# learningmatter-mit/surface-sampling

Hardware: AMD Instinct MI355X
Metric: MC energy-evaluations/sec (SrTiO3(001) ~250-atom slabs, 3-model PaiNN ensemble E+F incl. neighbor list) (higher is better)
Workload: dtype f32 via fp16x2-split MFMA (3 products), fp32 accumulate; neighbor decisions f64; 1 GPU; SrTiO3(001) PaiNN x3, 256 batched independent chains per GPU (BASELINE configs[3]), 248-272 atoms/chain; chains_per_gpu=256, atoms_per_gpu=66503, edges_per_gpu=2747786, slots_per_gpu=2836316, models=3, streams_per_gpu=2, parallelism=one GPU, no collective

## Files before the change

surface-sampling_amd/csrc/painn_edge_mfma.hip:

```cpp
#include "vssr_internal.h"

#ifdef EDGE_PHASE_TIMING
__device__ unsigned long long g_edge_phase[16];
#define EPH_INIT unsigned long long eph_acc[8] = {0, 0, 0, 0, 0, 0, 0, 0}, eph_t = wall_clock64();
#define EPH(k) { __builtin_amdgcn_sched_barrier(0); const unsigned long long eph_n = wall_clock64(); eph_acc[k] += eph_n - eph_t; eph_t = eph_n; __builtin_amdgcn_sched_barrier(0); }
#define EPH_FLUSH(base) if ((threadIdx.x & 63) == 0) { for (int q_ = 0; q_ < 8; ++q_) atomicAdd(&g_edge_phase[(base) + q_], eph_acc[q_]); }
extern "C" int vssr_debug_edge_phases(unsigned long long *out, int reset) {
    if (hipMemcpyFromSymbol(out, HIP_SYMBOL(g_edge_phase), sizeof(unsigned long long) * 16) != hipSuccess) return -1;
    if (reset) { unsigned long long z[16] = {}; if (hipMemcpyToSymbol(HIP_SYMBOL(g_edge_phase), z, sizeof(z)) != hipSuccess) return -1; }
    return 0;
}
#else
#define EPH_INIT
#define EPH(k)
#define EPH_FLUSH(base)
#endif

#ifndef SUB16_WAVES
#define SUB16_WAVES 12
#endif

namespace vssr {

typedef float f32x4 __attribute__((ext_vector_type(4)));

typedef unsigned u32x4 __attribute__((ext_vector_type(4)));
typedef _Float16 f16x8 __attribute__((ext_vector_type(8)));

__device__ __forceinline__ void mfma_pre_fence(u32x4 &a, u32x4 &b) {
    asm volatile("; mfma_pre_fence" : "+v"(a), "+v"(b) : : "memory");
}
__device__ __forceinline__ void arrival_fence(u32x4 &a, u32x4 &b) {
    asm volatile("; arrival_fence" : "+v"(a), "+v"(b) : : "memory");
}
__device__ __forceinline__ void arrival_fence(u32x4 &a, u32x4 &b, u32x4 &c, u32x4 &d, float &g) {
    asm volatile("; arrival_fence" : "+v"(a), "+v"(b), "+v"(c), "+v"(d), "+v"(g) : : "memory");
}
__device__ __forceinline__ float take(float src) {
    float d;
    asm("v_mov_b32 %0, %1" : "=v"(d) : "v"(src));
    return d;
}
__device__ __forceinline__ unsigned take_u(unsigned src) {
    unsigned d;
    asm("v_mov_b32 %0, %1" : "=v"(d) : "v"(src));
    return d;
}
__device__ __forceinline__ void mfma_load_fence(int &index, float &a, float &b, float &c) {
    asm volatile("; mfma_load_fence" : "+v"(index), "+v"(a), "+v"(b), "+v"(c));
}
// ... 54 lines not shown
    const auto hi = __builtin_amdgcn_permlane16_swap(a[1], a[1], false, false);
    s0 = __uint_as_float(lo[0]); s1 = __uint_as_float(lo[1]); s2 = __uint_as_float(hi[0]); s3 = __uint_as_float(hi[1]);
}

void build_wd16(const float *Wd, const float *bd, unsigned *dst) {
    auto split2 = [](float x, unsigned (&p)[2]) {
        const _Float16 h = (_Float16)x;
        const _Float16 l = (_Float16)(x - (float)h);
        unsigned short hb, lb;
        memcpy(&hb, &h, 2);
        memcpy(&lb, &l, 2);
        p[0] = hb; p[1] = lb;
    };
    for (int row = 0; row < F3; ++row)
        for (int kq = 0; kq < 4; ++kq) {
            unsigned wh[5], wl[5], bp[2];
            for (int t = 0; t < 5; ++t) {
                unsigned p2[2];
                split2(Wd[(size_t)row * 20 + kq + 4 * t], p2);
                wh[t] = p2[0]; wl[t] = p2[1];
            }
            split2(bd[row], bp);
            const unsigned bias = kq == 1 ? bp[1] : kq == 3 ? 0u : bp[0];
            const unsigned a1[8] = {wh[0], wh[1], wh[2], wh[3], wh[4], bias, wl[0], wl[1]};
            const unsigned a2[8] = {wl[2], wl[3], wl[4], wh[4], wh[0], wh[1], wh[2], wh[3]};
            unsigned *o = dst + ((size_t)row * 4 + kq) * 8;
            for (int q = 0; q < 4; ++q) {
                o[q] = a1[2 * q] | (a1[2 * q + 1] << 16);
                o[4 + q] = a2[2 * q] | (a2[2 * q + 1] << 16);
            }
        }
}

#ifndef STAGE_BATCH
#define STAGE_BATCH 4
#endif

template <int N> struct FeatVec { typedef float type __attribute__((ext_vector_type(N))); };
struct FeatVec1 {
    float v;
    __device__ __forceinline__ float operator[](int) const { return v; }
};
template <> struct FeatVec<1> { typedef FeatVec1 type; };

template <int NF>
struct EdgeGeo {
    static_assert(NF == 4 || NF == 2 || NF == 1, "16-, 8- or 4-feature slices");
    static constexpr int FS = 4 * NF;
    static constexpr int NSLICE = F / FS;
    static constexpr int NSEC = 3;
    static constexpr int NT = NF == 4 ? 3 : NF == 2 ? 2 : 1;
    static constexpr int NSEG = 6;
    static constexpr int ROW = NSEG * FS + 4;
    static constexpr int ROWB = FS * 4 + 4;
    __host__ __device__ static constexpr int row_section(int T, int i) {
        return NF == 4 ? T : NF == 1 ? ((i & 3) < 3 ? (i & 3) : -1) : (2 * T + ((i & 3) >> 1) < 3 ? 2 * T + ((i & 3) >> 1) : -1);
    }
    __host__ __device__ static constexpr int row_feature(int i) { return NF == 4 ? i : NF == 1 ? (i >> 2) : 2 * (i >> 2) + (i & 1); }
};
template <int NF> __device__ __forceinline__ constexpr int sec_tile(int sec) { return NF == 4 ? sec : NF == 1 ? 0 : sec >> 1; }
template <int NF> __device__ __forceinline__ constexpr int sec_reg(int sec, int r) { return NF == 4 ? r : NF == 1 ? sec : 2 * (sec & 1) + r; }

template <int NF, bool SLDS>
size_t edge_fwd_lds_bytes_t(int max_atoms) {
    return sizeof(float) * ((size_t)max_atoms * (EdgeGeo<NF>::ROW + (SLDS ? EdgeGeo<NF>::FS : 0)) + 4);
}

typedef float f32x2v __attribute__((ext_vector_type(2)));
// ... 20 lines not shown
}
template <int NF>
__device__ __forceinline__ void quad_sum_n(float (&x)[NF]) {
#pragma unroll
    for (int r = 0; r < NF; ++r) x[r] = quad_sum(x[r]);
    if constexpr (NF == 4) asm volatile("" : "+v"(x[0]), "+v"(x[1]), "+v"(x[2]), "+v"(x[3]));
    else if constexpr (NF == 2) asm volatile("" : "+v"(x[0]), "+v"(x[1]));
    else asm volatile("" : "+v"(x[0]));
}
template <int NF>
__device__ __forceinline__ void store_feat(float *dst, const float (&v)[NF]) {
    if constexpr (NF == 4) *reinterpret_cast<float4 *>(dst) = make_float4(v[0], v[1], v[2], v[3]);
    else if constexpr (NF == 2) *reinterpret_cast<float2 *>(dst) = make_float2(v[0], v[1]);
    else *dst = v[0];
}

__device__ __forceinline__ float xrow_sum(float x) {
    const unsigned u = __float_as_uint(x);
    const auto r32 = __builtin_amdgcn_permlane32_swap(u, u, false, false);
    const float y = __uint_as_float(r32[0]) + __uint_as_float(r32[1]);
    const unsigned v = __float_as_uint(y);
    const auto r16 = __builtin_amdgcn_permlane16_swap(v, v, false, false);
    return __uint_as_float(r16[0]) + __uint_as_float(r16[1]);
}

template <int NW>
struct BundleWalk {
    const int4 *tab;
    int Nc, wave, st;
    int nj;
    int j, t, Lc, Ln;
    int4 cur, nxt, pend;
    bool pend_ok;

    __device__ __forceinline__ int bundle_of(int jj) const { return jj * NW + ((jj & 1) ? NW - 1 - wave : wave); }
    __device__ __forceinline__ int4 load(int jj, bool &ok) const {
        const int idx = 4 * bundle_of(jj) + st;
        ok = jj < nj && idx < Nc;
        return tab[max(min(idx, Nc - 1), 0)];
    }
    __device__ __forceinline__ static int4 select(const int4 &v, bool ok) { return ok ? v : make_int4(-1, 0, 0, 0); }
    __device__ __forceinline__ static int steps(const int4 &q) { return max(__builtin_amdgcn_readfirstlane(q.z) >> 2, 2); }
    __device__ __forceinline__ void init(const int4 *table, int n, int w, int stream) {
        tab = table; Nc = n; wave = w; st = stream;
#ifdef ABL_NO_TAIL
        const int NB0 = (n + 3) >> 2, NB = NB0 >= NW ? NB0 - NB0 % NW : NB0, full = NB / NW, rem = NB - full * NW;
#else
        const int NB = (n + 3) >> 2, full = NB / NW, rem = NB - full * NW;
#endif
        nj = full + ((((full & 1) ? NW - 1 - w : w) < rem) ? 1 : 0);
        j = 0; t = 0;
        bool ok0, ok1;
        const int4 r0 = load(0, ok0), r1 = load(1, ok1);
        pend = load(2, pend_ok);
        cur = select(r0, ok0); nxt = select(r1, ok1);
        Lc = steps(cur); Ln = steps(nxt);
    }
    __device__ __forceinline__ int quad_ahead(int ahead, bool &valid) const {
        const int tt = t + ahead;
        const bool in_cur = tt < Lc;
        const int4 &q = in_cur ? cur : nxt;
        const int ts = in_cur ? tt : tt - Lc;
        valid = 4 * ts < q.z;
        return q.y + 4 * ts;
    }
    __device__ __forceinline__ void advance() {
        ++j;
        cur = nxt; nxt = select(pend, pend_ok);
        pend = load(j + 2, pend_ok);
        t = 0; Lc = Ln; Ln = steps(nxt);
    }
};

__device__ __forceinline__ int chain_of_workgroup(const GraphView &G, const int *__restrict__ list, int n_list, int per_chain, int &t) {
    const int wg = blockIdx.x, xcd = wg & 7, rest = wg >> 3;
    t = rest % per_chain;
    const int k = (rest / per_chain) * 8 + xcd;
    if (k >= n_list) return -1;
    const int b = list ? list[k] : k;
    return G.act.chain(b) ? b : -1;
}

template <bool ALIASED> struct EdgeOut { typedef float *__restrict__ ptr; };
template <> struct EdgeOut<true> { typedef float *ptr; };

template <int NF, bool SLDS, int WAVES, bool SUB = false>
__global__ void __launch_bounds__(64 * WAVES) __attribute__((amdgpu_waves_per_eu((SUB && NF == 4) ? WAVES / 4 : 4, (SUB && NF == 4) ? WAVES / 4 : 4)))
k_edge_fwd_mfma(int N, int l, const ModelW *__restrict__ MW, GraphView G, const int *__restrict__ counters,
                int zero_slot, int n_models, int max_atoms, const int *__restrict__ list, int n_list,
                const float *__restrict__ s_in, const float *__restrict__ v_in, const float *__restrict__ phi,
                typename EdgeOut<SUB>::ptr s_msg, typename EdgeOut<SUB>::ptr v_msg, const int4 *__restrict__ bundle_tab,
                const int *__restrict__ n_entries_tab, int pass, int chunk_max) {
    using LY = EdgeGeo<NF>;
    constexpr int FS = LY::FS, NSLICE = LY::NSLICE, NT = LY::NT, EDGE_THREADS = 64 * WAVES;
    static_assert(!SUB || !SLDS, "the sub-range form takes its residuals from memory");
    extern __shared__ __attribute__((aligned(16))) float tile[];
    if (counters[2]) return;
    int t;
    const int b = chain_of_workgroup(G, list, n_list, NSLICE * n_models, t);
    if (b < 0) return;
    const int fs = t % NSLICE, m = t / NSLICE;
    const int a0 = G.cfg_start[b], Nc = G.cfg_start[b + 1] - a0;
    const size_t mN = (size_t)m * N;
    const int tid = threadIdx.x;
    int lo = 0, ns = Nc;
    if constexpr (SUB) {
        if (pass >= sub_passes(Nc, chunk_max)) return;
        const int chunk = sub_chunk(Nc, chunk_max);
        lo = pass * chunk;
        ns = min(chunk, Nc - lo);
    }
    const float *res_s = (SUB && pass) ? s_msg : s_in, *res_v = (SUB && pass) ? v_msg : v_in;

    float *s_tile = tile + (size_t)max_atoms * LY::ROW;
    {
        constexpr int Q4 = FS / 4;
        constexpr int PER_ATOM = (LY::NSEG + (SLDS ? 1 : 0)) * Q4;
        const int total = ns * PER_ATOM;
        if constexpr (SUB) {
            for (int k = tid; k < LY::ROW; k += EDGE_THREADS) tile[(size_t)ns * LY::ROW + k] = 0.f;
        }
        auto src_of = [&](int idx) -> const float * {
            int atom = idx / PER_ATOM, rem = idx - atom * PER_ATOM, seg = rem / Q4, q4 = rem % Q4;
            const size_t ga = mN + a0 + lo + atom;
            if (seg == LY::NSEG) return s_in + ga * F + fs * FS + q4 * 4;
            if (seg < 3) return phi + ga * F3 + seg * F + fs * FS + q4 * 4;
            return v_in + (ga * 3 + (seg - 3)) * F + fs * FS + q4 * 4;
        };
        auto put = [&](int idx, const float4 &val) {
            int atom = idx / PER_ATOM, rem = idx - atom * PER_ATOM, seg = rem / Q4, q4 = rem % Q4;
            if (seg == LY::NSEG) {
                *reinterpret_cast<float4 *>(s_tile + atom * FS + q4 * 4) = val;
            } else {
                float *dst = tile + atom * LY::ROW + (q4 * 4) * LY::NSEG + seg;
                dst[0] = val.x; dst[LY::NSEG] = val.y; dst[2 * LY::NSEG] = val.z; dst[3 * LY::NSEG] = val.w;
            }
        };
        for (int base = tid; base < total; base += STAGE_BATCH * EDGE_THREADS) {
            float4 v4[STAGE_BATCH];
#pragma unroll
            for (int u = 0; u < STAGE_BATCH; ++u) {
                const int idx = min(base + u * EDGE_THREADS, total - 1);
                v4[u] = *reinterpret_cast<const float4 *>(src_of(idx));
            }
#pragma unroll
            for (int u = 0; u < STAGE_BATCH; ++u)
                if (base + u * EDGE_THREADS < total) put(base + u * EDGE_THREADS, v4[u]);
        }
    }
    __syncthreads();

    const int lane = tid & 63, wave = tid >> 6, p = lane & 15, fq = lane >> 4, e = p & 3;
    const LayerW &W = MW[m].layer[l];
    u32x4 wA[NT][2];
#pragma unroll
    for (int T = 0; T < NT; ++T) {
        const int sec = LY::row_section(T, p);
        const int row = max(sec, 0) * F + fs * FS + LY::row_feature(p);
        const u32x4 *wsrc = reinterpret_cast<const u32x4 *>(W.wd16) + ((size_t)row * 4 + fq) * 2;
#pragma unroll
        for (int i3 = 0; i3 < 2; ++i3) wA[T][i3] = sec < 0 ? (u32x4){0u, 0u, 0u, 0u} : gload_u32x4(wsrc + i3);
    }

    BundleWalk<EDGE_THREADS / 64> bw;
    int n_entries = Nc;
    if constexpr (SUB) {
        if (pass) n_entries = n_entries_tab[(size_t)(pass - 1) * G.n_cfg + b];
    }
    bw.init((SUB ? bundle_tab : G.bundle) + a0, n_entries, __builtin_amdgcn_readfirstlane(wave), p >> 2);
    if (bw.nj == 0) return;
#ifdef ABL_STAGE_ONLY
    if (bw.nj > 0) return;
#endif
    float ds[NF], dvx[NF], dvy[NF], dvz[NF];
#pragma unroll
    for (int r = 0; r < NF; ++r) { ds[r] = 0.f; dvx[r] = 0.f; dvy[r] = 0.f; dvz[r] = 0.f; }
    const int fcol = fs * FS + NF * fq;
    typedef typename FeatVec<NF>::type fres;
    fres sres_cur, sres_nxt, vres_cur[SUB ? 3 : 1];
    auto load_residual = [&](int cc) {
        return *reinterpret_cast<const fres *>(res_s + (mN + a0 + min(max(cc, 0), Nc - 1)) * F + fcol);
    };
    auto load_residual_v = [&](int cc, int x) {
        return *reinterpret_cast<const fres *>(res_v + ((mN + a0 + min(max(cc, 0), Nc - 1)) * 3 + x) * F + fcol);
    };
    if (!SLDS) { sres_cur = load_residual(bw.cur.x); sres_nxt = load_residual(bw.nxt.x); }
    if constexpr (SUB) {
#pragma unroll
        for (int x = 0; x < 3; ++x) vres_cur[x] = load_residual_v(bw.cur.x, x);
    }

    const u32x4 *rho_lane = reinterpret_cast<const u32x4 *>(G.rho16) + fq * 4 + e;
    const int zero_quad = (zero_slot + 1) / 4 - 1;

    u32x4 rq[2][2];
    auto fetch = [&](int buf, int quad_first_slot, bool valid) {
#ifdef ABL_TABLE_L2
        const u32x4 *rp = rho_lane + (size_t)(valid ? ((quad_first_slot >> 2) & 511) : zero_quad) * 32;
#else
        const u32x4 *rp = rho_lane + (size_t)(unsigned)(valid ? (quad_first_slot >> 2) : zero_quad) * 32;
#endif
        rq[buf][0] = rp[0]; rq[buf][1] = rp[16];
    };
    {
        bool v0, v1;
        const int q0 = bw.quad_ahead(0, v0), q1 = bw.quad_ahead(1, v1);
        fetch(0, q0, v0);
        __builtin_amdgcn_sched_barrier(0);
        fetch(1, q1, v1);
    }

    auto flush_bundle = [&]() {
        quad_sum_n<NF>(ds); quad_sum_n<NF>(dvx); quad_sum_n<NF>(dvy); quad_sum_n<NF>(dvz);
        const int c = bw.cur.x;
        if (e == 0 && c >= 0) {
            const size_t ga = mN + a0 + c;
            float so[NF], xo[NF], yo[NF], zo[NF];
            const float *sr = s_tile + c * FS + NF * fq;
            const float *vc = tile + c * LY::ROW + (NF * fq) * LY::NSEG;
#pragma unroll
            for (int r = 0; r < NF; ++r) {
                so[r] = ds[r] + (SLDS ? sr[r] : sres_cur[r]);
                xo[r] = dvx[r] + (SUB ? vres_cur[0][r] : vc[r * LY::NSEG + 3]);
                yo[r] = dvy[r] + (SUB ? vres_cur[SUB ? 1 : 0][r] : vc[r * LY::NSEG + 4]);
                zo[r] = dvz[r] + (SUB ? vres_cur[SUB ? 2 : 0][r] : vc[r * LY::NSEG + 5]);
            }
            store_feat<NF>(s_msg + ga * F + fcol, so);
            store_feat<NF>(v_msg + (ga * 3 + 0) * F + fcol, xo);
            store_feat<NF>(v_msg + (ga * 3 + 1) * F + fcol, yo);
            store_feat<NF>(v_msg + (ga * 3 + 2) * F + fcol, zo);
        }
#pragma unroll
        for (int r = 0; r < NF; ++r) { ds[r] = 0.f; dvx[r] = 0.f; dvy[r] = 0.f; dvz[r] = 0.f; }
    };

    lds_cfloat *trow = lds_base(tile) + (NF * fq) * LY::NSEG;
    EPH_INIT
    EPH(0)
    while (bw.j < bw.nj) {
#pragma unroll
        for (int ph = 0; ph < 2; ++ph) {
            arrival_fence(rq[ph][0], rq[ph][1]);
            EPH(1)
#ifdef ABL_LDS_BCAST
            const int jn = (int)(rq[ph][0][3] >> 16) & 1;
#else
            int jn = (int)rq[ph][1][3];
            if constexpr (SUB) {
                const unsigned jl = (unsigned)(jn - lo);
                jn = jl < (unsigned)ns ? (int)jl : ns;
            }
#endif
            if (bw.t == bw.Lc) {
                flush_bundle();
                bw.advance();
                if (!SLDS) {
                    sres_cur = sres_nxt;
                    __builtin_amdgcn_sched_barrier(0);
                    sres_nxt = load_residual(bw.nxt.x);
                    if constexpr (SUB) {
#pragma unroll
                        for (int x = 0; x < 3; ++x) vres_cur[x] = load_residual_v(bw.cur.x, x);
                    }
                }
                EPH(2)
            }
            float tv[NF * LY::NSEG];
            {
                if constexpr ((NF * LY::NSEG) % 4 == 0) {
// ... 50 lines not shown
#else
#pragma unroll
            for (int r = 1; r < NF; ++r) message(r);
#endif
            ++bw.t;
            EPH(6)
        }
    }
    EPH_FLUSH(0)
}

template <int NF, int WAVES>
constexpr int cen_floats() { return WAVES * 4 * 4 * 6 * NF; }
template <int NF, int WAVES>
#ifdef ABL_LDS_FORCE
size_t edge_bwd_lds_bytes_t(int max_atoms) { return sizeof(float) * ((size_t)max_atoms * EdgeGeo<NF>::ROWB + cen_floats<NF, WAVES>()) + 24 * (size_t)max_atoms + 32; }
#else
size_t edge_bwd_lds_bytes_t(int max_atoms) { return sizeof(float) * ((size_t)max_atoms * EdgeGeo<NF>::ROWB + cen_floats<NF, WAVES>()); }
#endif

template <int NF, bool FIRST, int WAVES, bool SUB = false>
__global__ void __launch_bounds__(64 * WAVES) __attribute__((amdgpu_waves_per_eu(2, 2)))
k_edge_bwd_mfma(int N, int l, const ModelW *__restrict__ MW, GraphView G,
                const int *__restrict__ counters, int zero_slot, int n_models, int max_atoms,
                const int *__restrict__ list, int n_list,
                const float *__restrict__ v_in, const float *__restrict__ phi, const float *__restrict__ sbar_msg,
                const float *__restrict__ vbar_msg, typename EdgeOut<SUB>::ptr phibar, typename EdgeOut<SUB>::ptr vbar_in,
                float *__restrict__ gbar, long long gbar_stride, int n_groups, int group_off, int rec,
                const int4 *__restrict__ bundle_tab, const int *__restrict__ n_entries_tab, int pass, int chunk_max) {
    using LY = EdgeGeo<NF>;
    constexpr int FS = LY::FS, NSG = LY::NSLICE, NT = LY::NT, ROWB = LY::ROWB, BWD_THREADS = 64 * WAVES;
    typedef typename FeatVec<NF>::type fvx;
    extern __shared__ __attribute__((aligned(16))) float tile[];
    if (counters[2]) return;
    int t;
    const int b = chain_of_workgroup(G, list, n_list, NSG * n_models, t);
    if (b < 0) return;
    const int fs = t % NSG, m = t / NSG;
    const int a0 = G.cfg_start[b], Nc = G.cfg_start[b + 1] - a0;
    const size_t mN = (size_t)m * N;
    const int tid = threadIdx.x;
    int lo = 0, ns = Nc;
    if constexpr (SUB) {
        if (pass >= sub_passes(Nc, chunk_max)) return;
        const int chunk = sub_chunk(Nc, chunk_max);
        lo = pass * chunk;
        ns = min(chunk, Nc - lo);
    }
    const int lane = tid & 63, wave = tid >> 6, p = lane & 15, fq = lane >> 4, e = p & 3;
    const int last_slot = max(G.row_start[a0 + Nc] - 1, 0);
    const LayerW &W = MW[m].layer[l];
    const int rec_c = FIRST ? 3 : rec;
    float *gb = gbar + (size_t)(m * n_groups + group_off + fs) * gbar_stride * rec_c;
    const u32x4 *rho_lane = reinterpret_cast<const u32x4 *>(G.rho16) + fq * 4 + e;
    const u32x4 *drho_lane = reinterpret_cast<const u32x4 *>(G.drho16) + fq * 4 + e;
    const int zero_quad = (zero_slot + 1) / 4 - 1;
    const int fcol = fs * FS + NF * fq;

    int gcomp_id;
    {
        unsigned t0 = 0u, t1 = 1u, t2 = 2u, t3 = 3u;
        asm volatile("" : "+v"(t0), "+v"(t1), "+v"(t2), "+v"(t3));
        const auto a = __builtin_amdgcn_permlane32_swap(t0, t1, false, false);
        const auto bq = __builtin_amdgcn_permlane32_swap(t2, t3, false, false);
        const auto cq = __builtin_amdgcn_permlane16_swap(a[0], bq[0], false, false);
        gcomp_id = (a[0] == a[1] && bq[0] == bq[1] && cq[0] == cq[1]) ? (int)cq[0] : 3;
        if (!(a[0] == a[1] && bq[0] == bq[1] && cq[0] == cq[1])) __builtin_trap();
    }

    {
        constexpr int Q4 = FS / 4;
        const int total = ns * 4 * Q4;
        if constexpr (SUB) {
            for (int k = tid; k < ROWB; k += BWD_THREADS) tile[(size_t)ns * ROWB + k] = 0.f;
        }
        for (int base = tid; base < total; base += STAGE_BATCH * BWD_THREADS) {
            float4 v4[STAGE_BATCH];
#pragma unroll
            for (int u = 0; u < STAGE_BATCH; ++u) {
                const int idx = min(base + u * BWD_THREADS, total - 1);
                const int atom = idx / (4 * Q4), seg = (idx / Q4) & 3, q4 = idx % Q4;
                const size_t ga = mN + a0 + lo + atom;
                const float *src = seg == 0 ? sbar_msg + ga * F + fs * FS + q4 * 4
                                            : vbar_msg + (ga * 3 + (seg - 1)) * F + fs * FS + q4 * 4;
                v4[u] = *reinterpret_cast<const float4 *>(src);
            }
#pragma unroll
            for (int u = 0; u < STAGE_BATCH; ++u) {
                const int idx = base + u * BWD_THREADS;
                if (idx < total) {
                    const int atom = idx / (4 * Q4), seg = (idx / Q4) & 3, q4 = idx % Q4;
                    float *dst = tile + atom * ROWB + (q4 * 4) * 4 + seg;
                    dst[0] = v4[u].x; dst[4] = v4[u].y; dst[8] = v4[u].z; dst[12] = v4[u].w;
                }
            }
        }
    }
    u32x4 wA[NT][2];
#pragma unroll
    for (int T = 0; T < NT; ++T) {
        const int sec = LY::row_section(T, p);
        const int row = max(sec, 0) * F + fs * FS + LY::row_feature(p);
        const u32x4 *wsrc = reinterpret_cast<const u32x4 *>(W.wd16) + ((size_t)row * 4 + fq) * 2;
#pragma unroll
        for (int i3 = 0; i3 < 2; ++i3) wA[T][i3] = sec < 0 ? (u32x4){0u, 0u, 0u, 0u} : gload_u32x4(wsrc + i3);
    }
#ifdef ABL_LDS_FORCE
    unsigned long long *facc = reinterpret_cast<unsigned long long *>(tile + (((size_t)max_atoms * ROWB + cen_floats<NF, WAVES>() + 1) & ~(size_t)1));
    for (int i = tid; i < 3 * Nc + 3; i += BWD_THREADS) facc[i] = 0ull;
    float gown = 0.f;
#endif
    __syncthreads();

    BundleWalk<BWD_THREADS / 64> bw;
    int n_entries = Nc;
    if constexpr (SUB) {
        if (pass) n_entries = n_entries_tab[(size_t)(pass - 1) * G.n_cfg + b];
    }
    bw.init((SUB ? bundle_tab : G.bundle) + a0, n_entries, __builtin_amdgcn_readfirstlane(wave), p >> 2);
    if (bw.nj == 0) return;
#ifdef ABL_STAGE_ONLY
    if (bw.nj > 0) return;
#endif

    const int cen_idx = max_atoms * ROWB + ((wave * 4 + (p >> 2)) * 4 + fq) * 6 * NF;
    fvx *cen = reinterpret_cast<fvx *>(tile + cen_idx);
    fvx nx[6];
    auto load_centre = [&](int cc) {
        const size_t ga = mN + a0 + min(max(cc, 0), Nc - 1);
        const float *pr = phi + ga * F3 + fcol;
        nx[0] = *reinterpret_cast<const fvx *>(pr);
        nx[1] = *reinterpret_cast<const fvx *>(pr + F);
        nx[2] = *reinterpret_cast<const fvx *>(pr + 2 * F);
        nx[3] = *reinterpret_cast<const fvx *>(v_in + (ga * 3 + 0) * F + fcol);
        nx[4] = *reinterpret_cast<const fvx *>(v_in + (ga * 3 + 1) * F + fcol);
        nx[5] = *reinterpret_cast<const fvx *>(v_in + (ga * 3 + 2) * F + fcol);
    };
    auto park_centre = [&]() {
#pragma unroll
        for (int q = 0; q < 6; ++q) cen[q] = nx[q];
    };
    load_centre(bw.cur.x);
    park_centre();
    load_centre(bw.nxt.x);
    fvx rres[SUB ? 6 : 1];
    auto load_rres = [&](int cc) {
        const size_t ga = mN + a0 + min(max(cc, 0), Nc - 1);
        const float *vsrc = pass ? vbar_in : vbar_msg;
#pragma unroll
        for (int x = 0; x < 3; ++x) rres[SUB ? 3 + x : 0] = *reinterpret_cast<const fvx *>(vsrc + (ga * 3 + x) * F + fcol);
        if (pass) {
#pragma unroll
            for (int q = 0; q < 3; ++q) rres[SUB ? q : 0] = *reinterpret_cast<const fvx *>(phibar + ga * F3 + q * F + fcol);
        }
    };
    if constexpr (SUB) load_rres(bw.cur.x);
    float accb[NF], accc[NF], accx[NF], accy[NF], accz[NF];
#pragma unroll
    for (int r = 0; r < NF; ++r) { accb[r] = 0.f; accc[r] = 0.f; accx[r] = 0.f; accy[r] = 0.f; accz[r] = 0.f; }

    auto flush_bundle = [&]() {
        quad_sum_n<NF>(accb); quad_sum_n<NF>(accc); quad_sum_n<NF>(accx); quad_sum_n<NF>(accy); quad_sum_n<NF>(accz);
        const float (&tb)[NF] = accb, (&tc)[NF] = accc, (&tx)[NF] = accx, (&ty)[NF] = accy, (&tz)[NF] = accz;
        const int c = bw.cur.x;
#ifdef ABL_LDS_FORCE
        {
            const float go = quad_sum(gown);
            gown = 0.f;
            if (e == 0 && c >= 0 && gcomp_id < 3)
                atomicAdd(&facc[3 * c + gcomp_id], (unsigned long long)__float2ll_rn(go * 4294967296.f));
        }
#endif
        if (e == 0 && c >= 0) {
            const size_t ga = mN + a0 + c;
            const fvx cv[6] = {cen[0], cen[1], cen[2], cen[3], cen[4], cen[5]};
            float a_[NF], x_[NF], y_[NF], z_[NF];
            const float *res = tile + c * ROWB + (NF * fq) * 4;
#pragma unroll
            for (int r = 0; r < NF; ++r) {
                a_[r] = fmaf(cv[5][r], tz[r], fmaf(cv[4][r], ty[r], cv[3][r] * tx[r]));
                x_[r] = fmaf(cv[0][r], tx[r], SUB ? rres[SUB ? 3 : 0][r] : res[4 * r + 1]);
                y_[r] = fmaf(cv[0][r], ty[r], SUB ? rres[SUB ? 4 : 0][r] : res[4 * r + 2]);
                z_[r] = fmaf(cv[0][r], tz[r], SUB ? rres[SUB ? 5 : 0][r] : res[4 * r + 3]);
            }
            float *pbp = phibar + ga * F3 + fcol;
            if (SUB && pass) {
                float b_[NF], c_[NF];
#pragma unroll
                for (int r = 0; r < NF; ++r) { a_[r] += rres[0][r]; b_[r] = tb[r] + rres[SUB ? 1 : 0][r]; c_[r] = tc[r] + rres[SUB ? 2 : 0][r]; }
                store_feat<NF>(pbp, a_);
                store_feat<NF>(pbp + F, b_);
                store_feat<NF>(pbp + 2 * F, c_);
            } else {
            store_feat<NF>(pbp, a_);
            store_feat<NF>(pbp + F, tb);
            store_feat<NF>(pbp + 2 * F, tc);
            }
            store_feat<NF>(vbar_in + (ga * 3 + 0) * F + fcol, x_);
            store_feat<NF>(vbar_in + (ga * 3 + 1) * F + fcol, y_);
            store_feat<NF>(vbar_in + (ga * 3 + 2) * F + fcol, z_);
        }
#pragma unroll
        for (int r = 0; r < NF; ++r) { accb[r] = 0.f; accc[r] = 0.f; accx[r] = 0.f; accy[r] = 0.f; accz[r] = 0.f; }
    };

    float *gcomp = gb + min(gcomp_id, rec_c - 1);
    u32x4 rq[2][2], dq[2][2];
    float gold[2] = {0.f, 0.f};
    auto fetch = [&](int buf, int quad_first_slot, bool valid) {
#ifdef ABL_TABLE_L2
        const size_t off = (size_t)(valid ? ((quad_first_slot >> 2) & 511) : zero_quad) * 32;
#else
        const size_t off = (size_t)(unsigned)(valid ? (quad_first_slot >> 2) : zero_quad) * 32;
#endif
        const u32x4 *rp = rho_lane + off, *dp = drho_lane + off;
        rq[buf][0] = rp[0]; rq[buf][1] = rp[16];
#ifdef ABL_3LOADS
        dq[buf][0] = dp[0]; dq[buf][1] = dq[buf][0];
#else
        dq[buf][0] = dp[0]; dq[buf][1] = dp[16];
#endif
#ifdef ABL_NO_GBAR
        if (!FIRST) gold[buf] = gcomp[(size_t)min((quad_first_slot + e) & 1023, last_slot) * rec_c];
#else
        if (!FIRST) gold[buf] = gcomp[(size_t)min(quad_first_slot + e, last_slot) * rec_c];
#endif
    };
    {
        bool v0, v1;
        const int q0 = bw.quad_ahead(0, v0), q1 = bw.quad_ahead(1, v1);
        fetch(0, q0, v0);
        __builtin_amdgcn_sched_barrier(0);
        fetch(1, q1, v1);
    }
    lds_cfloat *trow = lds_base(tile) + (NF * fq) * 4;
    EPH_INIT
    EPH(0)
    while (bw.j < bw.nj) {
#pragma unroll
        for (int ph = 0; ph < 2; ++ph) {
            arrival_fence(rq[ph][0], rq[ph][1], dq[ph][0], dq[ph][1], gold[ph]);
            EPH(1)
            bool in_range = true;
#ifdef ABL_LDS_BCAST
            const int jn = (int)(rq[ph][0][3] >> 16) & 1;
#else
            int jn = (int)rq[ph][1][3];
            if constexpr (SUB) {
                const unsigned jl = (unsigned)(jn - lo);
                in_range = jl < (unsigned)ns;
                jn = in_range ? (int)jl : ns;
            }
#endif
            const float gold_cur = FIRST ? 0.f : take(gold[ph]);
            if (bw.t == bw.Lc) {
                flush_bundle();
                bw.advance();
                park_centre();
                __builtin_amdgcn_sched_barrier(0);
                load_centre(bw.nxt.x);
                if constexpr (SUB) load_rres(bw.cur.x);
                EPH(2)
            }
            bool real_slot;
            const int my_slot = bw.quad_ahead(0, real_slot) + e;
            float tb[4 * NF];
            {
                lds_cfloat *row = lds_row(trow, jn, ROWB);
#pragma unroll
                for (int q = 0; q < NF; ++q) {
                    const f32x4 t4 = lds_read4(row + 4 * q);
                    tb[4 * q] = t4[0]; tb[4 * q + 1] = t4[1]; tb[4 * q + 2] = t4[2]; tb[4 * q + 3] = t4[3];
                }
            }
            fvx cv[6];
            {
                int ci = cen_idx;
                asm volatile("" : "+v"(ci));
                const fvx *cr = reinterpret_cast<const fvx *>(tile + ci);
#pragma unroll
                for (int q = 0; q < 6; ++q) cv[q] = cr[q];
            }
            float ux, uy, uz, invd;
            slot_scalars(take_u(rq[ph][1][2]), ux, uy, uz, invd);
            u32x4 rb2 = dense_b2(rq[ph][0], rq[ph][1]), db2 = dense_b2(dq[ph][0], dq[ph][1]);
            mfma_pre_fence(rq[ph][0], rb2);
            mfma_pre_fence(dq[ph][0], db2);
            EPH(3)
            f32x4 awd[2 * NT];
            {
                const u32x4 (*wp[2 * NT])[2], *bp1[2 * NT], *bp2[2 * NT];
#pragma unroll
                for (int s2 = 0; s2 < NT; ++s2) {
// ... 195 lines not shown
```

Baseline: 24530 evaluations/s.

## Overlap edge-kernel prologue loads with LDS staging and merge head lookups

Restructures the prologue of the forward and backward edge MFMA kernels. The weight loads, bundle-table loads, centre/residual loads and first rho/drho fetches are now all issued before the LDS staging stores and the barrier, so their latency overlaps the staging. The first staging batch is enlarged (8 fwd, 18 bwd) and issued up front. The workgroup head combines the stop flag, chain index, weight pointer and cfg_start lookups into fewer dependent rounds made wave-uniform via readfirstlane. Optional prologue clock instrumentation is added. The trade-off is higher register pressure from holding more in-flight loads, which could hurt occupancy.

Measured after the change: 24470 evaluations/s. No clear change (-0.2%).

```diff
diff --git a/surface-sampling_amd/csrc/painn_edge_mfma.hip b/surface-sampling_amd/csrc/painn_edge_mfma.hip
--- a/surface-sampling_amd/csrc/painn_edge_mfma.hip
+++ b/surface-sampling_amd/csrc/painn_edge_mfma.hip
@@ -16,6 +16,25 @@
 #define EPH_FLUSH(base)
 #endif
 
+#ifdef EDGE_PROLOGUE_CLOCKS
+__device__ unsigned long long g_edge_prologue[16];
+enum { EPC_ENTRY = 0, EPC_CHAIN, EPC_STAGED, EPC_BARRIER, EPC_WEIGHTS, EPC_BUNDLE, EPC_TABLE };
+#define EPC_INIT unsigned long long epc[7] = {0, 0, 0, 0, 0, 0, 0};
+#define EPC(k) { __builtin_amdgcn_sched_barrier(0); epc[k] = wall_clock64(); __builtin_amdgcn_sched_barrier(0); }
+#define EPC_USE4(x) asm volatile("; prologue clock: data used" : "+v"(x) : : "memory");
+#define EPC_FLUSH(base) if ((threadIdx.x & 63) == 0) { for (int q_ = 1; q_ < 7; ++q_) atomicAdd(&g_edge_prologue[(base) + q_], epc[q_] - epc[0]); atomicAdd(&g_edge_prologue[(base) + 7], 1ull); }
+extern "C" int vssr_debug_edge_prologue(unsigned long long *out, int reset) {
+    if (hipMemcpyFromSymbol(out, HIP_SYMBOL(g_edge_prologue), sizeof(unsigned long long) * 16) != hipSuccess) return -1;
+    if (reset) { unsigned long long z[16] = {}; if (hipMemcpyToSymbol(HIP_SYMBOL(g_edge_prologue), z, sizeof(z)) != hipSuccess) return -1; }
+    return 0;
+}
+#else
+#define EPC_INIT
+#define EPC(k)
+#define EPC_USE4(x)
+#define EPC_FLUSH(base)
+#endif
+
 #ifndef SUB16_WAVES
 #define SUB16_WAVES 12
 #endif
@@ -136,8 +155,14 @@
         }
 }
 
-#ifndef STAGE_BATCH
-#define STAGE_BATCH 4
+#ifndef STAGE_BATCH_FWD
+#define STAGE_BATCH_FWD 8
+#endif
+#ifndef STAGE_BATCH_BWD
+#define STAGE_BATCH_BWD 18
+#endif
+#ifndef STAGE_BATCH_MORE
+#define STAGE_BATCH_MORE 4
 #endif
 
 template <int N> struct FeatVec { typedef float type __attribute__((ext_vector_type(N))); };
@@ -224,6 +249,7 @@
     int j, t, Lc, Ln;
     int4 cur, nxt, pend;
     bool pend_ok;
+    bool cur_ok, nxt_ok;
 
     __device__ __forceinline__ int bundle_of(int jj) const { return jj * NW + ((jj & 1) ? NW - 1 - wave : wave); }
     __device__ __forceinline__ int4 load(int jj, bool &ok) const {
@@ -233,7 +259,7 @@
     }
     __device__ __forceinline__ static int4 select(const int4 &v, bool ok) { return ok ? v : make_int4(-1, 0, 0, 0); }
     __device__ __forceinline__ static int steps(const int4 &q) { return max(__builtin_amdgcn_readfirstlane(q.z) >> 2, 2); }
-    __device__ __forceinline__ void init(const int4 *table, int n, int w, int stream) {
+    __device__ __forceinline__ void issue(const int4 *table, int n, int w, int stream) {
         tab = table; Nc = n; wave = w; st = stream;
 #ifdef ABL_NO_TAIL
         const int NB0 = (n + 3) >> 2, NB = NB0 >= NW ? NB0 - NB0 % NW : NB0, full = NB / NW, rem = NB - full * NW;
@@ -242,10 +268,11 @@
 #endif
         nj = full + ((((full & 1) ? NW - 1 - w : w) < rem) ? 1 : 0);
         j = 0; t = 0;
-        bool ok0, ok1;
-        const int4 r0 = load(0, ok0), r1 = load(1, ok1);
+        cur = load(0, cur_ok); nxt = load(1, nxt_ok);
         pend = load(2, pend_ok);
-        cur = select(r0, ok0); nxt = select(r1, ok1);
+    }
+    __device__ __forceinline__ void finish() {
+        cur = select(cur, cur_ok); nxt = select(nxt, nxt_ok);
         Lc = steps(cur); Ln = steps(nxt);
     }
     __device__ __forceinline__ int quad_ahead(int ahead, bool &valid) const {
@@ -264,13 +291,30 @@
     }
 };
 
-__device__ __forceinline__ int chain_of_workgroup(const GraphView &G, const int *__restrict__ list, int n_list, int per_chain, int &t) {
-    const int wg = blockIdx.x, xcd = wg & 7, rest = wg >> 3;
-    t = rest % per_chain;
-    const int k = (rest / per_chain) * 8 + xcd;
-    if (k >= n_list) return -1;
-    const int b = list ? list[k] : k;
-    return G.act.chain(b) ? b : -1;
+__device__ __forceinline__ void head_trip(int &a, int &b, unsigned &c, unsigned &d) {
+    asm("; head trip" : "+v"(a), "+v"(b), "+v"(c), "+v"(d));
+    a = __builtin_amdgcn_readfirstlane(a); b = __builtin_amdgcn_readfirstlane(b);
+    c = __builtin_amdgcn_readfirstlane(c); d = __builtin_amdgcn_readfirstlane(d);
+}
+__device__ __forceinline__ bool workgroup_head(const GraphView &G, const int *__restrict__ counters, const int *__restrict__ list, int n_list,
+                                               int nslice, int n_models, const ModelW *__restrict__ MW, int l,
+                                               int &b, int &fs, int &m, int &a0, int &Nc, const uint4 *&wd16) {
+    const int wg = blockIdx.x, xcd = wg & 7, rest = wg >> 3, per_chain = nslice * n_models;
+    const int t = rest % per_chain, k = (rest / per_chain) * 8 + xcd;
+    fs = t % nslice; m = t / nslice;
+    const int kc = min(k, n_list - 1);
+    int stop = counters[2];
+    b = list ? list[kc] : kc;
+    const uintptr_t wp = reinterpret_cast<uintptr_t>(MW[m].layer[l].wd16);
+    unsigned wlo = (unsigned)wp, whi = (unsigned)(wp >> 32);
+    head_trip(stop, b, wlo, whi);
+    wd16 = reinterpret_cast<const uint4 *>((uintptr_t)wlo | ((uintptr_t)whi << 32));
+    a0 = G.cfg_start[b];
+    int a1 = G.cfg_start[b + 1];
+    unsigned act = G.act.mask ? (unsigned)G.act.mask[b] : 1u, none = 0u;
+    head_trip(a0, a1, act, none);
+    Nc = a1 - a0;
+    return !stop && k < n_list && act != 0u && Nc > 0;
 }
 
 template <bool ALIASED> struct EdgeOut { typedef float *__restrict__ ptr; };
@@ -287,14 +331,14 @@
     constexpr int FS = LY::FS, NSLICE = LY::NSLICE, NT = LY::NT, EDGE_THREADS = 64 * WAVES;
     static_assert(!SUB || !SLDS, "the sub-range form takes its residuals from memory");
     extern __shared__ __attribute__((aligned(16))) float tile[];
-    if (counters[2]) return;
-    int t;
-    const int b = chain_of_workgroup(G, list, n_list, NSLICE * n_models, t);
-    if (b < 0) return;
-    const int fs = t % NSLICE, m = t / NSLICE;
-    const int a0 = G.cfg_start[b], Nc = G.cfg_start[b + 1] - a0;
+    EPC_INIT
+    EPC(EPC_ENTRY)
+    int b, fs, m, a0, Nc;
+    const uint4 *wd16;
+    if (!workgroup_head(G, counters, list, n_list, NSLICE, n_models, MW, l, b, fs, m, a0, Nc, wd16)) return;
     const size_t mN = (size_t)m * N;
     const int tid = threadIdx.x;
+    EPC(EPC_CHAIN)
     int lo = 0, ns = Nc;
     if constexpr (SUB) {
         if (pass >= sub_passes(Nc, chunk_max)) return;
@@ -303,70 +347,56 @@
         ns = min(chunk, Nc - lo);
     }
     const float *res_s = (SUB && pass) ? s_msg : s_in, *res_v = (SUB && pass) ? v_msg : v_in;
-
-    float *s_tile = tile + (size_t)max_atoms * LY::ROW;
-    {
-        constexpr int Q4 = FS / 4;
-        constexpr int PER_ATOM = (LY::NSEG + (SLDS ? 1 : 0)) * Q4;
-        const int total = ns * PER_ATOM;
-        if constexpr (SUB) {
-            for (int k = tid; k < LY::ROW; k += EDGE_THREADS) tile[(size_t)ns * LY::ROW + k] = 0.f;
-        }
-        auto src_of = [&](int idx) -> const float * {
-            int atom = idx / PER_ATOM, rem = idx - atom * PER_ATOM, seg = rem / Q4, q4 = rem % Q4;
-            const size_t ga = mN + a0 + lo + atom;
-            if (seg == LY::NSEG) return s_in + ga * F + fs * FS + q4 * 4;
-            if (seg < 3) return phi + ga * F3 + seg * F + fs * FS + q4 * 4;
-            return v_in + (ga * 3 + (seg - 3)) * F + fs * FS + q4 * 4;
-        };
-        auto put = [&](int idx, const float4 &val) {
-            int atom = idx / PER_ATOM, rem = idx - atom * PER_ATOM, seg = rem / Q4, q4 = rem % Q4;
-            if (seg == LY::NSEG) {
-                *reinterpret_cast<float4 *>(s_tile + atom * FS + q4 * 4) = val;
-            } else {
-                float *dst = tile + atom * LY::ROW + (q4 * 4) * LY::NSEG + seg;
-                dst[0] = val.x; dst[LY::NSEG] = val.y; dst[2 * LY::NSEG] = val.z; dst[3 * LY::NSEG] = val.w;
-            }
-        };
-        for (int base = tid; base < total; base += STAGE_BATCH * EDGE_THREADS) {
-            float4 v4[STAGE_BATCH];
-#pragma unroll
-            for (int u = 0; u < STAGE_BATCH; ++u) {
-                const int idx = min(base + u * EDGE_THREADS, total - 1);
-                v4[u] = *reinterpret_cast<const float4 *>(src_of(idx));
-            }
-#pragma unroll
-            for (int u = 0; u < STAGE_BATCH; ++u)
-                if (base + u * EDGE_THREADS < total) put(base + u * EDGE_THREADS, v4[u]);
-        }
-    }
-    __syncthreads();
-
     const int lane = tid & 63, wave = tid >> 6, p = lane & 15, fq = lane >> 4, e = p & 3;
-    const LayerW &W = MW[m].layer[l];
+
     u32x4 wA[NT][2];
 #pragma unroll
     for (int T = 0; T < NT; ++T) {
         const int sec = LY::row_section(T, p);
         const int row = max(sec, 0) * F + fs * FS + LY::row_feature(p);
-        const u32x4 *wsrc = reinterpret_cast<const u32x4 *>(W.wd16) + ((size_t)row * 4 + fq) * 2;
+        const u32x4 *wsrc = reinterpret_cast<const u32x4 *>(wd16) + ((size_t)row * 4 + fq) * 2;
 #pragma unroll
         for (int i3 = 0; i3 < 2; ++i3) wA[T][i3] = sec < 0 ? (u32x4){0u, 0u, 0u, 0u} : gload_u32x4(wsrc + i3);
     }
-
     BundleWalk<EDGE_THREADS / 64> bw;
     int n_entries = Nc;
     if constexpr (SUB) {
         if (pass) n_entries = n_entries_tab[(size_t)(pass - 1) * G.n_cfg + b];
     }
-    bw.init((SUB ? bundle_tab : G.bundle) + a0, n_entries, __builtin_amdgcn_readfirstlane(wave), p >> 2);
-    if (bw.nj == 0) return;
-#ifdef ABL_STAGE_ONLY
-    if (bw.nj > 0) return;
-#endif
-    float ds[NF], dvx[NF], dvy[NF], dvz[NF];
-#pragma unroll
-    for (int r = 0; r < NF; ++r) { ds[r] = 0.f; dvx[r] = 0.f; dvy[r] = 0.f; dvz[r] = 0.f; }
+    bw.issue((SUB ? bundle_tab : G.bundle) + a0, n_entries, __builtin_amdgcn_readfirstlane(wave), p >> 2);
+    __builtin_amdgcn_sched_barrier(0);
+
+    float *s_tile = tile + (size_t)max_atoms * LY::ROW;
+    constexpr int Q4 = FS / 4;
+    constexpr int PER_ATOM = (LY::NSEG + (SLDS ? 1 : 0)) * Q4;
+    const int total = ns * PER_ATOM;
+    auto src_of = [&](int idx) -> const float * {
+        int atom = idx / PER_ATOM, rem = idx - atom * PER_ATOM, seg = rem / Q4, q4 = rem % Q4;
+        const size_t ga = mN + a0 + lo + atom;
+        if (seg == LY::NSEG) return s_in + ga * F + fs * FS + q4 * 4;
+        if (seg < 3) return phi + ga * F3 + seg * F + fs * FS + q4 * 4;
+        return v_in + (ga * 3 + (seg - 3)) * F + fs * FS + q4 * 4;
+    };
+    auto put = [&](int idx, const float4 &val) {
+        int atom = idx / PER_ATOM, rem = idx - atom * PER_ATOM, seg = rem / Q4, q4 = rem % Q4;
+        if (seg == LY::NSEG) {
+            *reinterpret_cast<float4 *>(s_tile + atom * FS + q4 * 4) = val;
+        } else {
+            float *dst = tile + atom * LY::ROW + (q4 * 4) * LY::NSEG + seg;
+            dst[0] = val.x; dst[LY::NSEG] = val.y; dst[2 * LY::NSEG] = val.z; dst[3 * LY::NSEG] = val.w;
+        }
+    };
+    float4 v4[STAGE_BATCH_FWD];
+#pragma unroll
+    for (int u = 0; u < STAGE_BATCH_FWD; ++u)
+        v4[u] = *reinterpret_cast<const float4 *>(src_of(min(tid + u * EDGE_THREADS, total - 1)));
+    __builtin_amdgcn_sched_barrier(0);
+
+    bw.finish();
+#ifdef EDGE_PROLOGUE_CLOCKS
+    asm volatile("" : "+s"(bw.Lc), "+s"(bw.Ln));
+#endif
+    EPC(EPC_BUNDLE)
     const int fcol = fs * FS + NF * fq;
     typedef typename FeatVec<NF>::type fres;
     fres sres_cur, sres_nxt, vres_cur[SUB ? 3 : 1];
@@ -376,11 +406,6 @@
     auto load_residual_v = [&](int cc, int x) {
         return *reinterpret_cast<const fres *>(res_v + ((mN + a0 + min(max(cc, 0), Nc - 1)) * 3 + x) * F + fcol);
     };
-    if (!SLDS) { sres_cur = load_residual(bw.cur.x); sres_nxt = load_residual(bw.nxt.x); }
-    if constexpr (SUB) {
-#pragma unroll
-        for (int x = 0; x < 3; ++x) vres_cur[x] = load_residual_v(bw.cur.x, x);
-    }
 
     const u32x4 *rho_lane = reinterpret_cast<const u32x4 *>(G.rho16) + fq * 4 + e;
     const int zero_quad = (zero_slot + 1) / 4 - 1;
@@ -401,6 +426,42 @@
         __builtin_amdgcn_sched_barrier(0);
         fetch(1, q1, v1);
     }
+    if (!SLDS) { sres_cur = load_residual(bw.cur.x); sres_nxt = load_residual(bw.nxt.x); }
+    if constexpr (SUB) {
+#pragma unroll
+        for (int x = 0; x < 3; ++x) vres_cur[x] = load_residual_v(bw.cur.x, x);
+    }
+    __builtin_amdgcn_sched_barrier(0);
+
+    if constexpr (SUB) {
+        for (int k = tid; k < LY::ROW; k += EDGE_THREADS) tile[(size_t)ns * LY::ROW + k] = 0.f;
+    }
+#pragma unroll
+    for (int u = 0; u < STAGE_BATCH_FWD; ++u)
+        if (tid + u * EDGE_THREADS < total) put(tid + u * EDGE_THREADS, v4[u]);
+    for (int base = tid + STAGE_BATCH_FWD * EDGE_THREADS; base < total; base += STAGE_BATCH_MORE * EDGE_THREADS) {
+        float4 w4[STAGE_BATCH_MORE];
+#pragma unroll
+        for (int u = 0; u < STAGE_BATCH_MORE; ++u)
+            w4[u] = *reinterpret_cast<const float4 *>(src_of(min(base + u * EDGE_THREADS, total - 1)));
+#pragma unroll
+        for (int u = 0; u < STAGE_BATCH_MORE; ++u)
+            if (base + u * EDGE_THREADS < total) put(base + u * EDGE_THREADS, w4[u]);
+    }
+    EPC(EPC_STAGED)
+    __syncthreads();
+    EPC(EPC_BARRIER)
+#ifdef EDGE_PROLOGUE_CLOCKS
+    for (int T = 0; T < NT; ++T) { EPC_USE4(wA[T][0]) EPC_USE4(wA[T][1]) }
+#endif
+    EPC(EPC_WEIGHTS)
+    if (bw.nj == 0) return;
+#ifdef ABL_STAGE_ONLY
+    if (bw.nj > 0) return;
+#endif
+    float ds[NF], dvx[NF], dvy[NF], dvz[NF];
+#pragma unroll
+    for (int r = 0; r < NF; ++r) { ds[r] = 0.f; dvx[r] = 0.f; dvy[r] = 0.f; dvz[r] = 0.f; }
 
     auto flush_bundle = [&]() {
         quad_sum_n<NF>(ds); quad_sum_n<NF>(dvx); quad_sum_n<NF>(dvy); quad_sum_n<NF>(dvz);
@@ -427,6 +488,9 @@
     };
 
     lds_cfloat *trow = lds_base(tile) + (NF * fq) * LY::NSEG;
+    EPC_USE4(rq[0][0]) EPC_USE4(rq[0][1])
+    EPC(EPC_TABLE)
+    EPC_FLUSH(0)
     EPH_INIT
     EPH(0)
     while (bw.j < bw.nj) {
@@ -543,14 +607,14 @@
     constexpr int FS = LY::FS, NSG = LY::NSLICE, NT = LY::NT, ROWB = LY::ROWB, BWD_THREADS = 64 * WAVES;
     typedef typename FeatVec<NF>::type fvx;
     extern __shared__ __attribute__((aligned(16))) float tile[];
-    if (counters[2]) return;
-    int t;
-    const int b = chain_of_workgroup(G, list, n_list, NSG * n_models, t);
-    if (b < 0) return;
-    const int fs = t % NSG, m = t / NSG;
-    const int a0 = G.cfg_start[b], Nc = G.cfg_start[b + 1] - a0;
+    EPC_INIT
+    EPC(EPC_ENTRY)
+    int b, fs, m, a0, Nc;
+    const uint4 *wd16;
+    if (!workgroup_head(G, counters, list, n_list, NSG, n_models, MW, l, b, fs, m, a0, Nc, wd16)) return;
     const size_t mN = (size_t)m * N;
     const int tid = threadIdx.x;
+    EPC(EPC_CHAIN)
     int lo = 0, ns = Nc;
     if constexpr (SUB) {
         if (pass >= sub_passes(Nc, chunk_max)) return;
@@ -560,7 +624,6 @@
     }
     const int lane = tid & 63, wave = tid >> 6, p = lane & 15, fq = lane >> 4, e = p & 3;
     const int last_slot = max(G.row_start[a0 + Nc] - 1, 0);
-    const LayerW &W = MW[m].layer[l];
     const int rec_c = FIRST ? 3 : rec;
     float *gb = gbar + (size_t)(m * n_groups + group_off + fs) * gbar_stride * rec_c;
     const u32x4 *rho_lane = reinterpret_cast<const u32x4 *>(G.rho16) + fq * 4 + e;
@@ -579,93 +642,143 @@
         if (!(a[0] == a[1] && bq[0] == bq[1] && cq[0] == cq[1])) __builtin_trap();
     }
 
-    {
-        constexpr int Q4 = FS / 4;
-        const int total = ns * 4 * Q4;
-        if constexpr (SUB) {
-            for (int k = tid; k < ROWB; k += BWD_THREADS) tile[(size_t)ns * ROWB + k] = 0.f;
-        }
-        for (int base = tid; base < total; base += STAGE_BATCH * BWD_THREADS) {
-            float4 v4[STAGE_BATCH];
-#pragma unroll
-            for (int u = 0; u < STAGE_BATCH; ++u) {
-                const int idx = min(base + u * BWD_THREADS, total - 1);
-                const int atom = idx / (4 * Q4), seg = (idx / Q4) & 3, q4 = idx % Q4;
-                const size_t ga = mN + a0 + lo + atom;
-                const float *src = seg == 0 ? sbar_msg + ga * F + fs * FS + q4 * 4
-                                            : vbar_msg + (ga * 3 + (seg - 1)) * F + fs * FS + q4 * 4;
-                v4[u] = *reinterpret_cast<const float4 *>(src);
-            }
-#pragma unroll
-            for (int u = 0; u < STAGE_BATCH; ++u) {
-                const int idx = base + u * BWD_THREADS;
-                if (idx < total) {
-                    const int atom = idx / (4 * Q4), seg = (idx / Q4) & 3, q4 = idx % Q4;
-                    float *dst = tile + atom * ROWB + (q4 * 4) * 4 + seg;
-                    dst[0] = v4[u].x; dst[4] = v4[u].y; dst[8] = v4[u].z; dst[12] = v4[u].w;
-                }
-            }
-        }
-    }
     u32x4 wA[NT][2];
 #pragma unroll
     for (int T = 0; T < NT; ++T) {
         const int sec = LY::row_section(T, p);
         const int row = max(sec, 0) * F + fs * FS + LY::row_feature(p);
-        const u32x4 *wsrc = reinterpret_cast<const u32x4 *>(W.wd16) + ((size_t)row * 4 + fq) * 2;
+        const u32x4 *wsrc = reinterpret_cast<const u32x4 *>(wd16) + ((size_t)row * 4 + fq) * 2;
 #pragma unroll
         for (int i3 = 0; i3 < 2; ++i3) wA[T][i3] = sec < 0 ? (u32x4){0u, 0u, 0u, 0u} : gload_u32x4(wsrc + i3);
     }
+    BundleWalk<BWD_THREADS / 64> bw;
+    int n_entries = Nc;
+    if constexpr (SUB) {
+        if (pass) n_entries = n_entries_tab[(size_t)(pass - 1) * G.n_cfg + b];
+    }
+    bw.issue((SUB ? bundle_tab : G.bundle) + a0, n_entries, __builtin_amdgcn_readfirstlane(wave), p >> 2);
+    __builtin_amdgcn_sched_barrier(0);
+
+    constexpr int Q4 = FS / 4;
+    const int total = ns * 4 * Q4;
+    auto src_of = [&](int idx) -> const float * {
+        const int atom = idx / (4 * Q4), seg = (idx / Q4) & 3, q4 = idx % Q4;
+        const size_t ga = mN + a0 + lo + atom;
+        return seg == 0 ? sbar_msg + ga * F + fs * FS + q4 * 4 : vbar_msg + (ga * 3 + (seg - 1)) * F + fs * FS + q4 * 4;
+    };
+    auto put = [&](int idx, const float4 &val) {
+        const int atom = idx / (4 * Q4), seg = (idx / Q4) & 3, q4 = idx % Q4;
+        float *dst = tile + atom * ROWB + (q4 * 4) * 4 + seg;
+        dst[0] = val.x; dst[4] = val.y; dst[8] = val.z; dst[12] = val.w;
+    };
+    float4 v4[STAGE_BATCH_BWD];
+#pragma unroll
+    for (int u = 0; u < STAGE_BATCH_BWD; ++u)
+        v4[u] = *reinterpret_cast<const float4 *>(src_of(min(tid + u * BWD_THREADS, total - 1)));
+    __builtin_amdgcn_sched_barrier(0);
+
+    bw.finish();
+#ifdef EDGE_PROLOGUE_CLOCKS
+    asm volatile("" : "+s"(bw.Lc), "+s"(bw.Ln));
+#endif
+    EPC(EPC_BUNDLE)
+    const int cen_idx = max_atoms * ROWB + ((wave * 4 + (p >> 2)) * 4 + fq) * 6 * NF;
+    fvx *cen = reinterpret_cast<fvx *>(tile + cen_idx);
+    fvx nx[6];
+    auto load_centre = [&](fvx (&dst)[6], int cc) {
+        const size_t ga = mN + a0 + min(max(cc, 0), Nc - 1);
+        const float *pr = phi + ga * F3 + fcol;
+        dst[0] = *reinterpret_cast<const fvx *>(pr);
+        dst[1] = *reinterpret_cast<const fvx *>(pr + F);
+        dst[2] = *reinterpret_cast<const fvx *>(pr + 2 * F);
+        dst[3] = *reinterpret_cast<const fvx *>(v_in + (ga * 3 + 0) * F + fcol);
+        dst[4] = *reinterpret_cast<const fvx *>(v_in + (ga * 3 + 1) * F + fcol);
+        dst[5] = *reinterpret_cast<const fvx *>(v_in + (ga * 3 + 2) * F + fcol);
+    };
+    auto park_centre = [&](const fvx (&src)[6]) {
+#pragma unroll
+        for (int q = 0; q < 6; ++q) cen[q] = src[q];
+    };
+    fvx first[6];
+    load_centre(first, bw.cur.x);
+    load_centre(nx, bw.nxt.x);
+    fvx rres[SUB ? 6 : 1];
+    auto load_rres = [&](int cc) {
+        const size_t ga = mN + a0 + min(max(cc, 0), Nc - 1);
+        const float *vsrc = pass ? vbar_in : vbar_msg;
+#pragma unroll
+        for (int x = 0; x < 3; ++x) rres[SUB ? 3 + x : 0] = *reinterpret_cast<const fvx *>(vsrc + (ga * 3 + x) * F + fcol);
+        if (pass) {
+#pragma unroll
+            for (int q = 0; q < 3; ++q) rres[SUB ? q : 0] = *reinterpret_cast<const fvx *>(phibar + ga * F3 + q * F + fcol);
+        }
+    };
+    if constexpr (SUB) load_rres(bw.cur.x);
+
+    float *gcomp = gb + min(gcomp_id, rec_c - 1);
+    u32x4 rq[2][2], dq[2][2];
+    float gold[2] = {0.f, 0.f};
+    auto fetch = [&](int buf, int quad_first_slot, bool valid) {
+#ifdef ABL_TABLE_L2
+        const size_t off = (size_t)(valid ? ((quad_first_slot >> 2) & 511) : zero_quad) * 32;
+#else
+        const size_t off = (size_t)(unsigned)(valid ? (quad_first_slot >> 2) : zero_quad) * 32;
+#endif
+        const u32x4 *rp = rho_lane + off, *dp = drho_lane + off;
+        rq[buf][0] = rp[0]; rq[buf][1] = rp[16];
+#ifdef ABL_3LOADS
+        dq[buf][0] = dp[0]; dq[buf][1] = dq[buf][0];
+#else
+        dq[buf][0] = dp[0]; dq[buf][1] = dp[16];
+#endif
+#ifdef ABL_NO_GBAR
+        if (!FIRST) gold[buf] = gcomp[(size_t)min((quad_first_slot + e) & 1023, last_slot) * rec_c];
+#else
+        if (!FIRST) gold[buf] = gcomp[(size_t)min(quad_first_slot + e, last_slot) * rec_c];
+#endif
+    };
+    {
+        bool v0, v1;
+        const int q0 = bw.quad_ahead(0, v0), q1 = bw.quad_ahead(1, v1);
+        fetch(0, q0, v0);
+        __builtin_amdgcn_sched_barrier(0);
+        fetch(1, q1, v1);
+    }
+    __builtin_amdgcn_sched_barrier(0);
+
+    if constexpr (SUB) {
+        for (int k = tid; k < ROWB; k += BWD_THREADS) tile[(size_t)ns * ROWB + k] = 0.f;
+    }
+#pragma unroll
+    for (int u = 0; u < STAGE_BATCH_BWD; ++u)
+        if (tid + u * BWD_THREADS < total) put(tid + u * BWD_THREADS, v4[u]);
+    for (int base = tid + STAGE_BATCH_BWD * BWD_THREADS; base < total; base += STAGE_BATCH_MORE * BWD_THREADS) {
+        float4 w4[STAGE_BATCH_MORE];
+#pragma unroll
+        for (int u = 0; u < STAGE_BATCH_MORE; ++u)
+            w4[u] = *reinterpret_cast<const float4 *>(src_of(min(base + u * BWD_THREADS, total - 1)));
+#pragma unroll
+        for (int u = 0; u < STAGE_BATCH_MORE; ++u)
+            if (base + u * BWD_THREADS < total) put(base + u * BWD_THREADS, w4[u]);
+    }
+    park_centre(first);
+    EPC(EPC_STAGED)
 #ifdef ABL_LDS_FORCE
     unsigned long long *facc = reinterpret_cast<unsigned long long *>(tile + (((size_t)max_atoms * ROWB + cen_floats<NF, WAVES>() + 1) & ~(size_t)1));
     for (int i = tid; i < 3 * Nc + 3; i += BWD_THREADS) facc[i] = 0ull;
     float gown = 0.f;
 #endif
     __syncthreads();
-
-    BundleWalk<BWD_THREADS / 64> bw;
-    int n_entries = Nc;
-    if constexpr (SUB) {
-        if (pass) n_entries = n_entries_tab[(size_t)(pass - 1) * G.n_cfg + b];
-    }
-    bw.init((SUB ? bundle_tab : G.bundle) + a0, n_entries, __builtin_amdgcn_readfirstlane(wave), p >> 2);
+    EPC(EPC_BARRIER)
+#ifdef EDGE_PROLOGUE_CLOCKS
+    for (int T = 0; T < NT; ++T) { EPC_USE4(wA[T][0]) EPC_USE4(wA[T][1]) }
+#endif
+    EPC(EPC_WEIGHTS)
     if (bw.nj == 0) return;
 #ifdef ABL_STAGE_ONLY
     if (bw.nj > 0) return;
 #endif
 
-    const int cen_idx = max_atoms * ROWB + ((wave * 4 + (p >> 2)) * 4 + fq) * 6 * NF;
-    fvx *cen = reinterpret_cast<fvx *>(tile + cen_idx);
-    fvx nx[6];
-    auto load_centre = [&](int cc) {
-        const size_t ga = mN + a0 + min(max(cc, 0), Nc - 1);
-        const float *pr = phi + ga * F3 + fcol;
-        nx[0] = *reinterpret_cast<const fvx *>(pr);
-        nx[1] = *reinterpret_cast<const fvx *>(pr + F);
-        nx[2] = *reinterpret_cast<const fvx *>(pr + 2 * F);
-        nx[3] = *reinterpret_cast<const fvx *>(v_in + (ga * 3 + 0) * F + fcol);
-        nx[4] = *reinterpret_cast<const fvx *>(v_in + (ga * 3 + 1) * F + fcol);
-        nx[5] = *reinterpret_cast<const fvx *>(v_in + (ga * 3 + 2) * F + fcol);
-    };
-    auto park_centre = [&]() {
-#pragma unroll
-        for (int q = 0; q < 6; ++q) cen[q] = nx[q];
-    };
-    load_centre(bw.cur.x);
-    park_centre();
-    load_centre(bw.nxt.x);
-    fvx rres[SUB ? 6 : 1];
-    auto load_rres = [&](int cc) {
-        const size_t ga = mN + a0 + min(max(cc, 0), Nc - 1);
-        const float *vsrc = pass ? vbar_in : vbar_msg;
-#pragma unroll
-        for (int x = 0; x < 3; ++x) rres[SUB ? 3 + x : 0] = *reinterpret_cast<const fvx *>(vsrc + (ga * 3 + x) * F + fcol);
-        if (pass) {
-#pragma unroll
-            for (int q = 0; q < 3; ++q) rres[SUB ? q : 0] = *reinterpret_cast<const fvx *>(phibar + ga * F3 + q * F + fcol);
-        }
-    };
-    if constexpr (SUB) load_rres(bw.cur.x);
     float accb[NF], accc[NF], accx[NF], accy[NF], accz[NF];
 #pragma unroll
     for (int r = 0; r < NF; ++r) { accb[r] = 0.f; accc[r] = 0.f; accx[r] = 0.f; accy[r] = 0.f; accz[r] = 0.f; }
@@ -715,36 +828,10 @@
         for (int r = 0; r < NF; ++r) { accb[r] = 0.f; accc[r] = 0.f; accx[r] = 0.f; accy[r] = 0.f; accz[r] = 0.f; }
     };
 
-    float *gcomp = gb + min(gcomp_id, rec_c - 1);
-    u32x4 rq[2][2], dq[2][2];
-    float gold[2] = {0.f, 0.f};
-    auto fetch = [&](int buf, int quad_first_slot, bool valid) {
-#ifdef ABL_TABLE_L2
-        const size_t off = (size_t)(valid ? ((quad_first_slot >> 2) & 511) : zero_quad) * 32;
-#else
-        const size_t off = (size_t)(unsigned)(valid ? (quad_first_slot >> 2) : zero_quad) * 32;
-#endif
-        const u32x4 *rp = rho_lane + off, *dp = drho_lane + off;
-        rq[buf][0] = rp[0]; rq[buf][1] = rp[16];
-#ifdef ABL_3LOADS
-        dq[buf][0] = dp[0]; dq[buf][1] = dq[buf][0];
-#else
-        dq[buf][0] = dp[0]; dq[buf][1] = dp[16];
-#endif
-#ifdef ABL_NO_GBAR
-        if (!FIRST) gold[buf] = gcomp[(size_t)min((quad_first_slot + e) & 1023, last_slot) * rec_c];
-#else
-        if (!FIRST) gold[buf] = gcomp[(size_t)min(quad_first_slot + e, last_slot) * rec_c];
-#endif
-    };
-    {
-        bool v0, v1;
-        const int q0 = bw.quad_ahead(0, v0), q1 = bw.quad_ahead(1, v1);
-        fetch(0, q0, v0);
-        __builtin_amdgcn_sched_barrier(0);
-        fetch(1, q1, v1);
-    }
     lds_cfloat *trow = lds_base(tile) + (NF * fq) * 4;
+    EPC_USE4(rq[0][0]) EPC_USE4(rq[0][1]) EPC_USE4(dq[0][0]) EPC_USE4(dq[0][1])
+    EPC(EPC_TABLE)
+    EPC_FLUSH(8)
     EPH_INIT
     EPH(0)
     while (bw.j < bw.nj) {
@@ -767,9 +854,9 @@
             if (bw.t == bw.Lc) {
                 flush_bundle();
                 bw.advance();
-                park_centre();
+                park_centre(nx);
                 __builtin_amdgcn_sched_barrier(0);
-                load_centre(bw.nxt.x);
+                load_centre(nx, bw.nxt.x);
                 if constexpr (SUB) load_rres(bw.cur.x);
                 EPH(2)
             }
```
